# scverse/scanpy

Hardware: AMD Instinct MI355X
Metric: cells/sec through pca+neighbors+leiden, 1M x 2k CSR (higher is better)
Workload: dtype bf16x3

## Files before the change

### include/scanpy_amd.h

```cpp
#ifndef SCANPY_AMD_H
#define SCANPY_AMD_H

#include <stddef.h>
#include <stdint.h>

#ifdef __cplusplus
extern "C" {
#endif

typedef struct ihipStream_t* scamd_stream_t;

#define SCAMD_OK 0
#define SCAMD_EINVAL (-1)
#define SCAMD_EWORKSPACE (-2)
#define SCAMD_EHIP (-3)
#define SCAMD_EUNSUPPORTED (-4)
#define SCAMD_ECAPACITY (-5)
#define SCAMD_EINTERNAL (-6)

#define SCAMD_ABI_VERSION 1

int scamd_abi_version(void);
const char* scamd_last_error(void);
int scamd_device_count(void);
// ... 5 lines not shown
                     double cert_scale, int64_t* n_fallback_host,
                     void* workspace, size_t workspace_bytes, scamd_stream_t stream);
int scamd_knn_l2_ivf_f32(const float* x, int64_t n, int d, int64_t ld_x,
                         int64_t q_begin, int64_t n_query, int k, int nprobe,
                         int32_t* out_idx, double* out_dist, int64_t* n_fallback_host,
                         void* workspace, size_t workspace_bytes, scamd_stream_t stream);
float scamd_knn_last_select_ms(void);
double scamd_knn_last_select_pairs(void);
double scamd_knn_last_select_prepass_pairs(void);
int scamd_knn_last_select_engine(void);
int scamd_knn_last_second_tier_queries(void);
int scamd_knn_last_nprobe(void);
int scamd_knn_last_coarse(void);
void scamd_knn_cert_factors(int engine, double* cert_k, double* cert_k2, double* key_slack);
size_t scamd_knn_debug_b3_scores_workspace_bytes(int64_t n);
int scamd_knn_debug_b3_scores_f32(const float* x, int64_t n, int d, int64_t ld_x, int64_t q0, int nq, int64_t c0, int nc,
                                  float* out_scores, float* out_mu, float* out_cmax, void* workspace,
                                  size_t workspace_bytes, scamd_stream_t stream);
int scamd_knn_debug_cell_tables_sizes(int64_t n, int d, int64_t n_query, int k, int nprobe, int* n_cells, int64_t* n_img_max);
int scamd_knn_debug_cell_tables(int64_t n, int d, int64_t n_query, int k, int nprobe, const void* workspace,
                                size_t workspace_bytes, int32_t* out_labels, int32_t* out_row_cell, int32_t* out_cell_map,
                                float* out_cent, float* out_radius, int32_t* out_tile0, int32_t* out_ntiles, int32_t* out_order,
                                float* out_lb2, int32_t* out_perm, int64_t* n_img_rows_host, scamd_stream_t stream);

size_t scamd_fuzzy_workspace_bytes(int64_t n, int k);
int scamd_fuzzy_simplicial_set_f32(const int32_t* knn_idx, const float* knn_dist, int64_t n, int k,
                                   int64_t* out_indptr, int32_t* out_indices, float* out_data,
                                   int64_t cap, float* out_sigma, float* out_rho, int64_t* nnz_host,
                                   void* workspace, size_t workspace_bytes, scamd_stream_t stream);
int scamd_fuzzy_weights_f32(const int32_t* knn_idx, const float* knn_dist, int64_t n_local, int k, int64_t row_begin,
                            int64_t n_total, const double* sum_all_dev, float* w, float* out_sigma, float* out_rho,
                            int32_t* out_count, scamd_stream_t stream);
size_t scamd_fuzzy_merge_workspace_bytes(int64_t n_local, int64_t cap);
int scamd_fuzzy_merge_rows_f32(const int32_t* knn_idx, const float* w, int64_t n_local, int k, const int64_t* in_indptr,
                               const int32_t* in_src, const float* in_w, int64_t* out_indptr, int32_t* out_indices,
                               float* out_data, int64_t cap, int64_t* nnz_host, void* workspace, size_t workspace_bytes,
                               scamd_stream_t stream);
int scamd_gauss_connectivities_f32(const int32_t* knn_idx, const float* knn_dist, int64_t n, int k, int64_t* out_indptr,
                                   int32_t* out_indices, float* out_data, int64_t cap, int64_t* nnz_host,
                                   void* workspace, size_t workspace_bytes, scamd_stream_t stream);
int scamd_jaccard_connectivities_f32(const int32_t* knn_idx, int64_t n, int k, int64_t* out_indptr,
                                     int32_t* out_indices, float* out_data, int64_t cap, int64_t* nnz_host,
                                     void* workspace, size_t workspace_bytes, scamd_stream_t stream);


int scamd_csr_row_stats_f32(const int64_t* indptr, const float* data, int64_t n_rows,
// ... 236 lines not shown
```

### scanpy_amd/_lib.py

```python
from __future__ import annotations

import ctypes as C
from functools import lru_cache
from pathlib import Path

LIB_PATH = Path(__file__).resolve().parent / "_lib" / "libscanpy_amd.so"

_i64, _i32, _f64, _sz, _vp, _u64 = C.c_int64, C.c_int, C.c_double, C.c_size_t, C.c_void_p, C.c_uint64

SIGNATURES = {
    "scamd_abi_version": (_i32, []),
    "scamd_last_error": (C.c_char_p, []),
    "scamd_device_count": (_i32, []),
    "scamd_knn_workspace_bytes": (_sz, [_i64, _i32, _i64, _i32]),
    "scamd_knn_l2_f32": (_i32, [_vp, _i64, _i32, _i64, _i64, _i64, _i32, _vp, _vp, _f64, C.POINTER(_i64), _vp, _sz, _vp]),
    "scamd_knn_l2_ivf_f32": (_i32, [_vp, _i64, _i32, _i64, _i64, _i64, _i32, _i32, _vp, _vp, C.POINTER(_i64), _vp, _sz, _vp]),
    "scamd_knn_last_select_ms": (C.c_float, []),
    "scamd_knn_last_select_pairs": (_f64, []),
    "scamd_knn_last_select_prepass_pairs": (_f64, []),
    "scamd_knn_last_select_engine": (_i32, []),
    "scamd_knn_last_second_tier_queries": (_i32, []),
    "scamd_knn_last_nprobe": (_i32, []),
    "scamd_knn_last_coarse": (_i32, []),
    "scamd_knn_cert_factors": (None, [_i32, C.POINTER(_f64), C.POINTER(_f64), C.POINTER(_f64)]),
    "scamd_knn_debug_b3_scores_workspace_bytes": (_sz, [_i64]),
    "scamd_knn_debug_b3_scores_f32": (_i32, [_vp, _i64, _i32, _i64, _i64, _i32, _i64, _i32, _vp, _vp, _vp, _vp, _sz, _vp]),
    "scamd_knn_debug_cell_tables_sizes": (_i32, [_i64, _i32, _i64, _i32, _i32, C.POINTER(_i32), C.POINTER(_i64)]),
    "scamd_knn_debug_cell_tables": (_i32, [_i64, _i32, _i64, _i32, _i32, _vp, _sz, _vp, _vp, _vp, _vp, _vp, _vp, _vp, _vp, _vp, _vp,
                                           C.POINTER(_i64), _vp]),
    "scamd_fuzzy_workspace_bytes": (_sz, [_i64, _i32]),
    "scamd_fuzzy_simplicial_set_f32": (_i32, [_vp, _vp, _i64, _i32, _vp, _vp, _vp, _i64, _vp, _vp, C.POINTER(_i64), _vp, _sz, _vp]),
    "scamd_fuzzy_weights_f32": (_i32, [_vp, _vp, _i64, _i32, _i64, _i64, _vp, _vp, _vp, _vp, _vp, _vp]),
    "scamd_fuzzy_merge_workspace_bytes": (_sz, [_i64, _i64]),
    "scamd_fuzzy_merge_rows_f32": (_i32, [_vp, _vp, _i64, _i32, _vp, _vp, _vp, _vp, _vp, _vp, _i64, C.POINTER(_i64), _vp, _sz, _vp]),
    "scamd_gauss_connectivities_f32": (_i32, [_vp, _vp, _i64, _i32, _vp, _vp, _vp, _i64, C.POINTER(_i64), _vp, _sz, _vp]),
    "scamd_jaccard_connectivities_f32": (_i32, [_vp, _i64, _i32, _vp, _vp, _vp, _i64, C.POINTER(_i64), _vp, _sz, _vp]),
    "scamd_csr_row_stats_f32": (_i32, [_vp, _vp, _i64, _vp, _vp, _vp]),
    "scamd_csr_transpose_workspace_bytes": (_sz, [_i64, _i64, _i64]),
    "scamd_csr_transpose_f32": (_i32, [_vp, _vp, _vp, _i64, _i64, _i64, _vp, _vp, _vp, _vp, _sz, _vp]),
    "scamd_spmm_csr_f32": (_i32, [_vp, _vp, _vp, _i64, _i64, _vp, _i32, _vp, _vp, _vp]),
    "scamd_spmm_f64acc_workspace_bytes": (_sz, [_i64, _i64, _i32]),
    "scamd_spmm_csr_f32_f64acc": (_i32, [_vp, _vp, _vp, _i64, _i64, _vp, _i32, _vp, _vp, _vp, _vp, _sz, _vp]),
    "scamd_csr_gram_workspace_bytes": (_sz, [_i64, _i64]),
    "scamd_csr_gram_f32": (_i32, [_vp, _vp, _vp, _i64, _i64, _i64, _i32, _vp, _i64, _vp, C.POINTER(C.c_float), _vp, _sz, _vp]),
    "scamd_eigh_topk_workspace_bytes": (_sz, [_i64, _i32]),
    "scamd_eigh_topk_f64": (_i32, [_vp, _i64, _i64, _i32, _u64, _f64, _vp, _vp, _vp, _vp, _sz, _vp]),
    "scamd_dense_debug_f64": (_i32, [_i32, _vp, _vp, _i32, _i32, _i32, _vp, _vp, C.POINTER(_i32), _vp]),
    "scamd_pca_csr_workspace_bytes": (_sz, [_i64, _i64, _i32]),
    "scamd_pca_csr_f32": (_i32, [_vp, _vp, _vp, _i64, _i64, _i64, _i32, _i32, _u64, _f64, _vp, _vp, _vp, _vp, _vp, _vp, _vp, _sz, _vp]),
    "scamd_pca_solve_gram_workspace_bytes": (_sz, [_i64, _i32]),
    "scamd_pca_solve_gram_f64": (_i32, [_vp, _i64, _vp, _i64, _i64, _i32, _i32, _i32, _u64, _f64, _vp, _vp, _vp, _vp, _vp, _vp, _vp, _vp, _vp, _sz, _vp]),
    "scamd_spectral_embedding_workspace_bytes": (_sz, [_i64, _i64, _i32]),
# ... 131 lines not shown
```

### scanpy_amd/csrc/knn.hip

```cpp
#include "common.h"

#include <algorithm>
#include <cmath>
#include <cstdlib>
#include <memory>
#include <type_traits>
#include <vector>

struct KnnLast {
  float select_ms = -1.f;
  double select_pairs = -1.0, select_prepass_pairs = -1.0;
  int select_engine = -1, second_tier = 0;
  int coarse = 0;
  int nprobe = 0;
};
static thread_local KnnLast g_last;

namespace scamd {

using f32x16 = __attribute__((ext_vector_type(16))) float;
using f32x4 = __attribute__((ext_vector_type(4))) float;
using i32x4 = __attribute__((ext_vector_type(4))) int;
typedef __attribute__((__vector_size__(8 * sizeof(__bf16)))) __bf16 bf16x8;

// ... 989 lines not shown
      } else {
        __syncthreads();
        if (threadIdx.x == 0) {
          int got = -1;
          const int x0 = (int)(blockIdx.x & 7);
          for (int t = 0; t < 8 && got < 0; ++t) {
            const int x = (x0 + t) & 7;
            const int64_t peek = 8 * (int64_t)__hip_atomic_load(&iv.queue_ctr[x], __ATOMIC_RELAXED, __HIP_MEMORY_SCOPE_AGENT) + x;
            if (peek >= iv.n_slots || iv.block_perm[peek] < 0) continue;
            const int64_t slot = 8 * (int64_t)atomicAdd(&iv.queue_ctr[x], 1) + x;
            if (slot < iv.n_slots) got = iv.block_perm[slot];
          }
          *s_next = got;
        }
        __syncthreads();
        blk = *s_next;
      }
      if (blk < 0) return;
      knn_select_reg_block<H, TC_, WPS, IVF, B3, COARSE>(blk, xp, n_tiles_all, n_pad, q_begin, thr_rank, cand_idx, cand_tau, iv);
    }
  }
}

__global__ __launch_bounds__(256) void ivf_cell_order_kernel(const float* __restrict__ centers, int d,
                                                             const float* __restrict__ radius,
                                                             const int* __restrict__ cell_ntiles, int n_cells,
                                                             int* __restrict__ order_out, float* __restrict__ lb2_out,
                                                             int* __restrict__ work_out, int nprobe) {
  extern __shared__ __attribute__((aligned(16))) float co_smem[];
  int npow = 1;
  while (npow < n_cells) npow <<= 1;
  float* lb2 = co_smem;
  int* order = reinterpret_cast<int*>(co_smem + npow);
  const int a = blockIdx.x, tid = threadIdx.x;
  const float ra = radius[a];
  for (int b = tid; b < npow; b += 256) {
    float v = INFINITY;
    if (b < n_cells && cell_ntiles[b] > 0) {
      float d2 = 0.f;
      for (int c = 0; c < d; ++c) {
        const float df = centers[a * d + c] - centers[b * d + c];
        d2 += df * df;
      }
      const float lb = fmaxf(0.f, sqrtf(d2) * (1.0f - 1e-4f) - ra - radius[b]);
      v = (b == a) ? -1.0f : (nprobe > 0 ? d2 : lb * lb);
    }
    lb2[b] = v;
    order[b] = b;
  }
  __syncthreads();
  for (int kk = 2; kk <= npow; kk <<= 1) {
    for (int j = kk >> 1; j > 0; j >>= 1) {
      for (int i = tid; i < npow; i += 256) {
        const int p = i ^ j;
        if (p > i) {
          const bool up = (i & kk) == 0;
          const float vi = lb2[i], vp = lb2[p];
          const int oi = order[i], op = order[p];
          const bool gt = vi > vp || (vi == vp && oi > op);
          if (gt == up) {
            lb2[i] = vp;
            lb2[p] = vi;
            order[i] = op;
            order[p] = oi;
          }
        }
      }
      __syncthreads();
    }
  }
  if (nprobe > 0) {
    for (int i = tid; i < npow; i += 256)
      if (i > 0) lb2[i] = (i < nprobe && lb2[i] < INFINITY) ? 0.f : INFINITY;
    __syncthreads();
  }
  for (int i = tid; i < n_cells; i += 256) {
    order_out[(int64_t)a * n_cells + i] = order[i];
    lb2_out[(int64_t)a * n_cells + i] = lb2[i];
  }
  __shared__ int s_work;
  if (tid == 0) s_work = 0;
  __syncthreads();
  int wsum = 0;
  for (int i = tid; i < n_cells; i += 256)
    if (lb2[i] <= ra * ra) wsum += cell_ntiles[order[i]];
  atomicAdd(&s_work, wsum);
  __syncthreads();
  if (tid == 0) work_out[a] = cell_ntiles[a] > 0 ? s_work : 0;
}

__global__ __launch_bounds__(1024) void ivf_block_order_kernel(const int* __restrict__ work, const int* __restrict__ blk_off,
                                                               const int* __restrict__ blk_cnt, int n_cells,
                                                               int* __restrict__ block_perm, int n_slots, int xcd_mode,
                                                               int* __restrict__ err) {
  __shared__ long long key[IVF_MAX_CELLS];
  __shared__ int start[IVF_MAX_CELLS];
  const int tid = threadIdx.x;
  start[tid] = -1;
  key[tid] = tid < n_cells ? (((long long)(0x7fffffff - work[tid])) << 32) | (unsigned int)tid : 0x7fffffffffffffffll;
  for (int t = tid; t < n_slots; t += 1024) block_perm[t] = -1;
  __syncthreads();
  for (int kk = 2; kk <= IVF_MAX_CELLS; kk <<= 1) {
    for (int j = kk >> 1; j > 0; j >>= 1) {
      const int p = tid ^ j;
      if (p > tid) {
        const bool up = (tid & kk) == 0;
        const long long a = key[tid], b = key[p];
        if ((a > b) == up) {
          key[tid] = b;
          key[p] = a;
        }
// ... 789 lines not shown
  p->n_cells = 0;
  p->n_img_max = p->n_slot_max = 0;
  if (p->ivf) {
    const int cell_rows = std::max(256, env_int("SCAMD_KNN_CELL_ROWS", 2048));
    int c = 16;
    while (c < IVF_MAX_CELLS && (int64_t)c * cell_rows < n) c <<= 1;
    while (c > 1 && (int64_t)c * 256 > n) c >>= 1;
    p->n_cells = c;
    p->n_img_max = (n + (int64_t)64 * c + 255) / 256 * 256;
    p->n_slot_max = n_query + (int64_t)128 * c;
    p->n_pad = p->n_img_max;
  }
  return true;
}

struct KnnBuffers {
  float* xp; float* cn; float* mu; double* mean_partial; unsigned int* cmax; int* cand_idx; float* cand_tau; double* kth_d2;
  int* flag_list; int* counters; double* scratch_d; int* scratch_i; int* fb_counts;
  int* fb_retry[2];
  int* kth_idx;
  int* labels; int* perm; int* qpos; int* block_cell; float* cent; float* centp; long long* sums; int* cell_ints;
  unsigned int* radius_bits; int* cell_order; float* cell_lb2; int* cell_aux; int* block_perm;
  int* qorder;
  int* qrow; float* xp2; int* flag_list2; int* t2_cell; int* t2_pos; int* t2_ints;
};

static size_t block_perm_capacity(const KnnPlan& p) { return (size_t)(p.n_slot_max / 128 + 1) * 2 + 64; }
static void knn_carve(Workspace& ws, const KnnPlan& p, int64_t n_query, KnnBuffers* b) {
  *b = KnnBuffers{};
  b->xp = ws.take<float>((size_t)p.n_pad * p.row_dwords);
  b->cn = ws.take<float>((size_t)p.n_pad);
  b->mu = ws.take<float>(KNN_MAX_D);
  b->mean_partial = ws.take<double>((size_t)MEAN_BLOCKS * KNN_MAX_D);
  b->cmax = ws.take<unsigned int>(4);
  b->cand_idx = ws.take<int>((size_t)p.nq_pad * p.KP);
  b->cand_tau = ws.take<float>((size_t)p.nq_pad);
  b->kth_d2 = ws.take<double>((size_t)n_query);
  b->flag_list = ws.take<int>((size_t)n_query);
  b->counters = ws.take<int>(16);
  b->scratch_d = ws.take<double>((size_t)FALLBACK_CHUNK * FALLBACK_CAP);
  b->scratch_i = ws.take<int>((size_t)FALLBACK_CHUNK * FALLBACK_CAP);
  b->fb_counts = ws.take<int>((size_t)FALLBACK_CHUNK);
  b->fb_retry[0] = ws.take<int>((size_t)n_query);
  b->fb_retry[1] = ws.take<int>((size_t)n_query);
  b->kth_idx = ws.take<int>((size_t)n_query);
  if (p.ivf) {
    b->labels = ws.take<int>((size_t)p.n_pad);
    b->perm = ws.take<int>((size_t)p.n_img_max);
    b->qpos = ws.take<int>((size_t)p.n_slot_max);
    b->block_cell = ws.take<int>((size_t)(p.n_slot_max / 128 + 1));
    b->cent = ws.take<float>((size_t)p.n_cells * 128);
    b->centp = ws.take<float>((size_t)p.n_cells * 136);
    b->sums = ws.take<long long>((size_t)p.n_cells * 128);
    b->cell_ints = ws.take<int>((size_t)p.n_cells * 8);
    b->radius_bits = ws.take<unsigned int>((size_t)p.n_cells);
    b->cell_order = ws.take<int>((size_t)p.n_cells * p.n_cells);
    b->cell_lb2 = ws.take<float>((size_t)p.n_cells * p.n_cells);
    b->cell_aux = ws.take<int>((size_t)p.n_cells * 3);
    b->block_perm = ws.take<int>(block_perm_capacity(p));
    b->qorder = ws.take<int>((size_t)p.n_slot_max);
  }
  if (p.ivf && p.b3) {
    b->qrow = ws.take<int>((size_t)n_query);
    b->xp2 = ws.take<float>((size_t)p.n_img_max * RegCfg<25>::DPL);
    b->flag_list2 = ws.take<int>((size_t)n_query);
    b->t2_cell = ws.take<int>((size_t)n_query);
    b->t2_pos = ws.take<int>((size_t)n_query);
    b->t2_ints = ws.take<int>((size_t)p.n_cells * 2 + 8);
  }
}

struct CellTables {
  int *counts, *qcounts;
  int* cell_map;
  int *row_off, *row_cur;
  int *slot_off, *slot_cur;
  int *tile0, *ntiles;
  const float* radius;
  int *work, *first_block, *n_blocks;
};
static CellTables cell_tables(const KnnBuffers& b, size_t nc) {
  int* const ci = b.cell_ints;
  int* const ca = b.cell_aux;
// ... 60 lines not shown
      case 16: return launch_select_reg<16>(p, b, q_begin, s);
      case 25: return launch_select_reg<25>(p, b, q_begin, s);
      default: return launch_select_reg<32>(p, b, q_begin, s);
    }
  }
  switch (p.H) {
    case 8: return dispatch_kp<8, 128>(p, b, q_begin, s);
    case 16: return dispatch_kp<16, 128>(p, b, q_begin, s);
    case 25: return dispatch_kp<25, 128>(p, b, q_begin, s);
    case 32: return dispatch_kp<32, 128>(p, b, q_begin, s);
    case 64: return dispatch_kp<64, 64>(p, b, q_begin, s);
    default: return dispatch_kp<128, 32>(p, b, q_begin, s);
  }
}

struct KnnCall { const float* x; int64_t n; int d; int64_t ld, q_begin, n_query; hipStream_t s;
                 int k; double cert_scale; int32_t* out_idx; double* out_dist; };
struct HipRelease {
  void operator()(hipEvent_t e) const { (void)hipEventDestroy(e); }
  void operator()(void* p) const { (void)hipFree(p); }
};
using EventOwner = std::unique_ptr<std::remove_pointer_t<hipEvent_t>, HipRelease>;

static IvfArgs ivf_args(const KnnBuffers& b, const CellTables& t, int n_cells, int d) {
  IvfArgs iv{};
  iv.qpos = b.qpos;
  iv.block_cell = b.block_cell;
  iv.cell_tile0 = t.tile0;
  iv.cell_ntiles = t.ntiles;
  iv.centers = b.cent;
  iv.radius = t.radius;
  iv.order = b.cell_order;
  iv.order_lb2 = b.cell_lb2;
  iv.perm = b.perm;
  iv.cmax_bits = b.cmax;
  iv.n_cells = n_cells;
  iv.dc = d;
  iv.d = d;
  iv.block_perm = b.block_perm;
  return iv;
}

static int64_t layout_query_blocks(const std::vector<int>& n_queries, std::vector<int>* slot_off, std::vector<int>* block_cell) {
  int64_t slots = 0;
  for (size_t c = 0; c < n_queries.size(); ++c) {
    slot_off->push_back((int)slots);
    const int nb = (n_queries[c] + 127) / 128;
    block_cell->insert(block_cell->end(), nb, (int)c);
    slots += (int64_t)nb * 128;
  }
  return slots;
}

struct CellLayout {
  std::vector<int> cell_map, row_off, slot_off, tile0, ntiles, block_cell;
  std::vector<int> blocks;
  int64_t rows = 0, slots = 0;
  int n_launch = 0, xcd_mode = 0;
};

static CellLayout ivf_cell_layout(const std::vector<int>& h_cnt, const std::vector<float>& h_cent, int nc, int d, size_t launch_cap) {
  constexpr int MIN_CELL = 128;
  CellLayout L;
  L.cell_map.resize(nc);
  std::vector<int> mc(nc, 0), mq(nc, 0);
  int biggest = 0;
  for (int c = 1; c < nc; ++c)
    if (h_cnt[c] > h_cnt[biggest]) biggest = c;
  for (int c = 0; c < nc; ++c) {
    int tgt = c;
    if (h_cnt[c] < MIN_CELL) {
      tgt = biggest;
      double bestd = INFINITY;
      for (int e = 0; e < nc; ++e) {
        if (h_cnt[e] < MIN_CELL) continue;
        double dd = 0.0;
        for (int t = 0; t < d; ++t) {
          const double df = (double)h_cent[(size_t)c * d + t] - (double)h_cent[(size_t)e * d + t];
          dd += df * df;
        }
        if (dd < bestd) {
          bestd = dd;
          tgt = e;
        }
      }
    }
    L.cell_map[c] = tgt;
    mc[tgt] += h_cnt[c];
    mq[tgt] += h_cnt[nc + c];
  }
  for (int c = 0; c < nc; ++c) {
    L.row_off.push_back((int)L.rows);
    L.tile0.push_back((int)(L.rows / 64));
    L.ntiles.push_back((mc[c] + 63) / 64);
    L.rows += (int64_t)L.ntiles[c] * 64;
  }
  L.slots = layout_query_blocks(mq, &L.slot_off, &L.block_cell);
  L.blocks.resize(2 * nc);
  int maxb = 0;
  for (int c = 0; c < nc; ++c) {
    L.blocks[c] = L.slot_off[c] / 128;
    L.blocks[nc + c] = (mq[c] + 127) / 128;
    maxb = std::max(maxb, L.blocks[nc + c]);
  }
  const int n_blocks = (int)L.block_cell.size();
  const int64_t want = (int64_t)8 * (2 * ((n_blocks + 7) / 8) + maxb);
  L.n_launch = n_blocks;
  if (n_blocks >= 64 && want <= (int64_t)launch_cap) {
    L.xcd_mode = 1;
    L.n_launch = (int)want;
  }
  return L;
}

struct IvfSelect {
  const KnnPlan& p;
  const KnnBuffers& b;
  const KnnCall& c;
  decltype(&ivf_assign_kernel<8>) assign_f32;
  decltype(&knn_select_reg_kernel<8, 64, 3, true, false>) sweep[2];
  size_t sweep_lds;
  const CellTables t = cell_tables(b, p.n_cells);
  const int nc = p.n_cells;
  bool mfma_assign = false;
  int ncp = 0;
  size_t lds_a = 0;
  int assign(int64_t a_start, int64_t a_step, int64_t a_count, int accumulate, int64_t aq0, int64_t aq1, int* a_qcounts,
             bool count_in_kernel = true) const {
    hipStream_t s = c.s;
    if (mfma_assign) {
      unsigned int* centb = reinterpret_cast<unsigned int*>(b.centp);
      hipLaunchKernelGGL(ivf_centpad_bf16_kernel, dim3((unsigned)ceil_div((int64_t)ncp * 32, 256)), dim3(256), 0, s, b.cent, nc, ncp, c.d,
                         centb);
      SCAMD_LAUNCH_CHECK();
      hipLaunchKernelGGL(ivf_assign_mfma_kernel, dim3((unsigned)ceil_div(a_count, ASSIGN_ROWS)), dim3(256), lds_a, s, c.x, c.d, c.ld, a_start,
                         a_step, a_count, centb, ncp, nc, b.labels, count_in_kernel ? t.counts : (int*)nullptr, aq0, aq1, a_qcounts);
      SCAMD_LAUNCH_CHECK();
      if (accumulate) {
        hipLaunchKernelGGL(ivf_sums_kernel, dim3((unsigned)ceil_div(a_count * c.d, 256)), dim3(256), 0, s, c.x, c.d, c.ld, a_start, a_step,
                           a_count, b.labels, b.sums);
        SCAMD_LAUNCH_CHECK();
      }
// ... 26 lines not shown
      hipLaunchKernelGGL(ivf_update_kernel, dim3((unsigned)ceil_div((int64_t)nc * c.d, 256)), dim3(256), 0, c.s, b.sums, t.counts, nc,
                         c.d, b.cent);
      SCAMD_LAUNCH_CHECK();
    }
    return SCAMD_OK;
  }
  int assign_rows(std::vector<int>* h_cnt, std::vector<float>* h_cent) const {
    SCAMD_HIP_CHECK(hipMemsetAsync(t.counts, 0, sizeof(int) * 2 * nc, c.s));
    if (int rc = assign(0, 1, c.n, 0, c.q_begin, c.q_begin + c.n_query, t.qcounts, !mfma_assign)) return rc;
    if (mfma_assign) {
      hipLaunchKernelGGL(ivf_count_kernel, dim3((unsigned)ceil_div(c.n, 4096)), dim3(1024), 0, c.s, b.labels, c.n, nc, c.q_begin,
                         c.q_begin + c.n_query, t.counts, t.qcounts);
      SCAMD_LAUNCH_CHECK();
    }
    SCAMD_HIP_CHECK(hipMemcpyAsync(h_cnt->data(), t.counts, sizeof(int) * 2 * nc, hipMemcpyDeviceToHost, c.s));
    SCAMD_HIP_CHECK(hipMemcpyAsync(h_cent->data(), b.cent, sizeof(float) * nc * c.d, hipMemcpyDeviceToHost, c.s));
    SCAMD_HIP_CHECK(hipStreamSynchronize(c.s));
    return SCAMD_OK;
  }
  int upload_tables(const CellLayout& L) const {
    hipStream_t s = c.s;
    const size_t cell_bytes = sizeof(int) * nc;
    const std::pair<int*, const std::vector<int>*> per_cell[] = {
        {t.cell_map, &L.cell_map}, {t.row_off, &L.row_off}, {t.slot_off, &L.slot_off}, {t.tile0, &L.tile0}, {t.ntiles, &L.ntiles}};
    for (const auto& [dst, src] : per_cell) SCAMD_HIP_CHECK(hipMemcpyAsync(dst, src->data(), cell_bytes, hipMemcpyHostToDevice, s));
    SCAMD_HIP_CHECK(hipMemcpyAsync(b.block_cell, L.block_cell.data(), sizeof(int) * L.block_cell.size(), hipMemcpyHostToDevice, s));
    SCAMD_HIP_CHECK(hipMemcpyAsync(t.first_block, L.blocks.data(), 2 * cell_bytes, hipMemcpyHostToDevice, s));
    SCAMD_HIP_CHECK(hipMemsetAsync(t.row_cur, 0, cell_bytes, s));
    SCAMD_HIP_CHECK(hipMemsetAsync(t.slot_cur, 0, cell_bytes, s));
    SCAMD_HIP_CHECK(hipMemsetAsync(b.perm, 0xff, sizeof(int) * L.rows, s));
    SCAMD_HIP_CHECK(hipMemsetAsync(b.qpos, 0xff, sizeof(int) * L.slots, s));
    SCAMD_HIP_CHECK(hipMemsetAsync(b.radius_bits, 0, sizeof(unsigned int) * nc, s));
    SCAMD_HIP_CHECK(hipMemsetAsync(b.counters + KC_PAIRS, 0, sizeof(int) * (KC_LAUNCH_ORDER_ERR - KC_PAIRS), s));
    SCAMD_HIP_CHECK(hipStreamSynchronize(s));
    return SCAMD_OK;
  }
  int build_image_and_orders(const CellLayout& L) const {
    hipStream_t s = c.s;
    hipLaunchKernelGGL(ivf_scatter_kernel, dim3((unsigned)ceil_div(c.n, 1024 * SCATTER_ROWS)), dim3(1024), 0, s, b.labels, c.n, t.cell_map,
                       t.row_off, t.row_cur, c.q_begin, c.q_begin + c.n_query, t.slot_off, t.slot_cur, b.perm, b.qpos, b.qrow, nc);
    SCAMD_LAUNCH_CHECK();
    const int blocks = (int)std::min<int64_t>((L.rows + 15) / 16, 256 * 16);
    hipLaunchKernelGGL(ivf_pack_image_kernel, dim3(blocks), dim3(256), 0, s, c.x, b.mu, c.d, c.ld, p.H, (p.H + 1 + 3) / 4 * 4, p.row_dwords, L.rows, b.perm, b.labels,
                       t.cell_map, b.cent, b.xp, b.cmax, b.radius_bits, p.b3 ? 1 : 0);
    SCAMD_LAUNCH_CHECK();
    int npow = 1;
    while (npow < nc) npow <<= 1;
    const size_t olds = (size_t)npow * 8;
    SCAMD_HIP_CHECK(hipFuncSetAttribute(reinterpret_cast<const void*>(ivf_cell_order_kernel),
                                        hipFuncAttributeMaxDynamicSharedMemorySize, (int)olds));
    hipLaunchKernelGGL(ivf_cell_order_kernel, dim3(nc), dim3(256), olds, s, b.cent, c.d, t.radius, t.ntiles, nc, b.cell_order, b.cell_lb2,
                       t.work, p.nprobe);
    SCAMD_LAUNCH_CHECK();
    hipLaunchKernelGGL(ivf_block_order_kernel, dim3(1), dim3(1024), 0, s, t.work, t.first_block, t.n_blocks, nc, b.block_perm, L.n_launch,
                       L.xcd_mode, b.counters + KC_LAUNCH_ORDER_ERR);
    SCAMD_LAUNCH_CHECK();
    return SCAMD_OK;
  }
  int choose_coarse(const CellLayout& L, bool* coarse) const {
    *coarse = p.b3 && env_is("SCAMD_KNN_COARSE", '1');
    if (!p.b3 || *coarse || env_is("SCAMD_KNN_COARSE", '0')) return SCAMD_OK;
    std::vector<int> h_work(nc);
    SCAMD_HIP_CHECK(hipMemcpyAsync(h_work.data(), t.work, sizeof(int) * nc, hipMemcpyDeviceToHost, c.s));
    SCAMD_HIP_CHECK(hipStreamSynchronize(c.s));
    double num = 0.0, den = 0.0;
    for (int cell = 0; cell < nc; ++cell) {
      num += (double)L.blocks[nc + cell] * (double)h_work[cell] * 64.0;
      den += (double)L.blocks[nc + cell];
    }
    *coarse = den > 0.0 && num / den >= 5.0e5;
    return SCAMD_OK;
  }
  int launch_sweep(const CellLayout& L, bool coarse, hipEvent_t ev0, hipEvent_t ev1) const {
    hipStream_t s = c.s;
    const size_t n_blocks = L.block_cell.size();
    const auto kern = sweep[coarse];
    const size_t lds = sweep_lds + 64 + IVF_META_BYTES;
    SCAMD_HIP_CHECK(hipFuncSetAttribute(reinterpret_cast<const void*>(kern), hipFuncAttributeMaxDynamicSharedMemorySize, (int)lds));
    IvfArgs iv = ivf_args(b, t, nc, c.d);
    iv.pairs = reinterpret_cast<unsigned long long*>(b.counters + KC_PAIRS);
    iv.qorder = b.qorder;
    iv.prepass_tiles = p.b3 ? 32 : 16;
    iv.prepass_min2 = env_is("SCAMD_KNN_PREPASS_MIN2", '0') ? 0 : 1;
    std::unique_ptr<void, HipRelease> trace;
    const char* trace_path = getenv("SCAMD_KNN_TRACE");
    if (trace_path && trace_path[0]) {
      SCAMD_HIP_CHECK(hipMalloc(reinterpret_cast<void**>(&iv.trace), sizeof(unsigned long long) * 8 * n_blocks));
      trace.reset(iv.trace);
      SCAMD_HIP_CHECK(hipMemsetAsync(iv.trace, 0, sizeof(unsigned long long) * 8 * n_blocks, s));
    }
    int n_groups = L.n_launch;
    iv.n_slots = L.n_launch;
    const int want = env_int("SCAMD_KNN_PERSISTENT", 768);
    if (want > 0 && L.n_launch > want) {
      n_groups = (want + 7) / 8 * 8;
      iv.queue_ctr = b.counters + KC_XCD_QUEUE;
      SCAMD_HIP_CHECK(hipMemsetAsync(b.counters + KC_XCD_QUEUE, 0, sizeof(int) * 8, s));
    }
    SCAMD_HIP_CHECK(hipEventRecord(ev0, s));
    hipLaunchKernelGGL(kern, dim3(n_groups), dim3(RegCfg<8>::NT), lds, s, b.xp, (int)(L.rows / 64), L.rows, c.q_begin, p.thr_rank,
                       b.cand_idx, b.cand_tau, iv);
    SCAMD_LAUNCH_CHECK();
// ... 14 lines not shown
  int run(hipEvent_t ev0, hipEvent_t ev1, int64_t* rows_out) {
    std::vector<int> h_cnt(2 * nc);
    std::vector<float> h_cent((size_t)nc * c.d);
    if (int rc = train_quantiser()) return rc;
    if (int rc = assign_rows(&h_cnt, &h_cent)) return rc;
    const CellLayout L = ivf_cell_layout(h_cnt, h_cent, nc, c.d, block_perm_capacity(p));
    SCAMD_REQUIRE(L.rows <= p.n_img_max && L.slots <= p.n_slot_max, SCAMD_EWORKSPACE, "knn: cell layout exceeds its bound");
    rows_out[0] = L.rows;
    rows_out[1] = L.slots;
    if (L.block_cell.empty()) return SCAMD_OK;
    if (int rc = upload_tables(L)) return rc;
    if (int rc = build_image_and_orders(L)) return rc;
    bool coarse = false;
    if (int rc = choose_coarse(L, &coarse)) return rc;
    g_last.coarse = coarse ? 1 : 0;
    return launch_sweep(L, coarse, ev0, ev1);
  }
};

template <int H, bool B3 = false>
static int run_ivf_select(const KnnPlan& p, const KnnBuffers& b, const KnnCall& c, hipEvent_t ev0, hipEvent_t ev1, int64_t* rows_out) {
  using C = RegCfg<H, 64, B3>;
  static_assert(C::NT == RegCfg<8>::NT, "every instantiation is launched with the same block size");
  IvfSelect sel{p, b, c, ivf_assign_kernel<H>,
                {knn_select_reg_kernel<H, 64, 3, true, B3>, knn_select_reg_kernel<H, 64, 3, true, B3, B3>}, C::LDS_BYTES};
  return sel.run(ev0, ev1, rows_out);
}

static int dispatch_ivf(const KnnPlan& p, const KnnBuffers& b, const KnnCall& c, hipEvent_t ev0, hipEvent_t ev1, int64_t* rows_out) {
  switch (p.H) {
    case 8: return run_ivf_select<8>(p, b, c, ev0, ev1, rows_out);
    case 16: return run_ivf_select<16>(p, b, c, ev0, ev1, rows_out);
    case 25: return p.b3 ? run_ivf_select<25, true>(p, b, c, ev0, ev1, rows_out) : run_ivf_select<25>(p, b, c, ev0, ev1, rows_out);
    default: return run_ivf_select<32>(p, b, c, ev0, ev1, rows_out);
  }
}

static int launch_rerank_rows(const KnnBuffers& b, const KnnCall& c, int thr_rank, double cert_k, double cert_k2, int* flag_list,
                              int* n_flag, const int* qlist, int64_t n_list) {
  const int n_rank = std::max(1, thr_rank - 1);
  const size_t lds = rerank_rows_lds_bytes(c.d, n_rank);
  SCAMD_HIP_CHECK(hipFuncSetAttribute(reinterpret_cast<const void*>(knn_rerank_rows_kernel),
                                      hipFuncAttributeMaxDynamicSharedMemorySize, (int)lds));
  hipLaunchKernelGGL(knn_rerank_rows_kernel, dim3((unsigned)ceil_div(n_list, 8)), dim3(256), lds, c.s, c.x, b.mu, c.n, c.d, c.ld,
                     c.q_begin, c.n_query, c.k, n_rank, b.cand_idx, b.cand_tau, b.cmax, c.cert_scale, cert_k, cert_k2, c.out_idx,
                     c.out_dist, b.kth_d2, flag_list, n_flag, qlist, n_list);
  SCAMD_LAUNCH_CHECK();
// ... 37 lines not shown
  const int n_blocks = (int)h_block_cell.size();
  if (n_blocks == 0) return SCAMD_OK;
  SCAMD_REQUIRE(slots <= p.n_slot_max, SCAMD_EWORKSPACE, "knn: second-tier query layout exceeds its bound");
  SCAMD_HIP_CHECK(hipMemcpyAsync(slot_off2, h_slot_off.data(), sizeof(int) * nc, hipMemcpyHostToDevice, s));
  SCAMD_HIP_CHECK(hipMemcpyAsync(b.block_cell, h_block_cell.data(), sizeof(int) * n_blocks, hipMemcpyHostToDevice, s));
  SCAMD_HIP_CHECK(hipMemsetAsync(b.qpos, 0xff, sizeof(int) * slots, s));
  SCAMD_HIP_CHECK(hipStreamSynchronize(s));
  hipLaunchKernelGGL(ivf_t2_fill_kernel, dim3((unsigned)ceil_div(n_flag, 256)), dim3(256), 0, s, b.flag_list, n_flag, b.t2_cell,
                     b.t2_pos, slot_off2, b.qrow, b.qpos);
  SCAMD_LAUNCH_CHECK();
  t2_dbg(s, __LINE__);
  hipLaunchKernelGGL(knn_iota_kernel, dim3((unsigned)ceil_div(n_blocks, 256)), dim3(256), 0, s, b.block_perm, n_blocks);
  SCAMD_LAUNCH_CHECK();
  t2_dbg(s, __LINE__);
  const int blocks = (int)std::min<int64_t>((rows + 3) / 4, 256 * 16);
  hipLaunchKernelGGL(ivf_pack_image_kernel, dim3(blocks), dim3(256), 0, s, c.x, b.mu, c.d, c.ld, 25, C::HP, C::DPL, rows, b.perm,
                     b.labels, t.cell_map, b.cent, b.xp2, b.cmax, b.radius_bits, 0);
  SCAMD_LAUNCH_CHECK();
  t2_dbg(s, __LINE__);
  auto kern = knn_select_reg_kernel<25, 64, 3, true, false>;
  const size_t lds = C::LDS_BYTES + 64 + IVF_META_BYTES;
  SCAMD_HIP_CHECK(hipFuncSetAttribute(reinterpret_cast<const void*>(kern), hipFuncAttributeMaxDynamicSharedMemorySize,
                                      (int)lds));
  IvfArgs iv = ivf_args(b, t, nc, c.d);
  iv.pairs = reinterpret_cast<unsigned long long*>(ctr2 + KC_PAIRS);
  iv.prepass_tiles = 16;
  iv.prepass_min2 = 1;
  iv.n_slots = n_blocks;
  const int thr_rank = std::min(32, std::max(1, c.k + 6));
  hipLaunchKernelGGL(kern, dim3(n_blocks), dim3(C::NT), lds, s, b.xp2, (int)(rows / 64), rows, c.q_begin, thr_rank, b.cand_idx,
                     b.cand_tau, iv);
  SCAMD_LAUNCH_CHECK();
  t2_dbg(s, __LINE__);
  if (int rc = launch_rerank_rows(b, c, thr_rank, CERT_K_F32, 0.0, b.flag_list2, ctr2 + KC_UNCERTIFIED, b.flag_list, n_flag)) return rc;
  t2_dbg(s, __LINE__);
  SCAMD_READBACK_NOW(n_flag2_host, ctr2 + KC_UNCERTIFIED, sizeof(int), s);
  return SCAMD_OK;
}

static int stage_mean_and_image(const KnnPlan& p, const KnnBuffers& b, const KnnCall& c) {
  hipStream_t s = c.s;
  SCAMD_HIP_CHECK(hipMemsetAsync(b.cmax, 0, 16, s));
  SCAMD_HIP_CHECK(hipMemsetAsync(b.counters, 0, sizeof(int) * KC_HOST_SLOTS, s));
  hipLaunchKernelGGL(knn_colsum_kernel, dim3(MEAN_BLOCKS), dim3(1024), 0, s, c.x, c.n, c.d, c.ld, b.mean_partial);
  SCAMD_LAUNCH_CHECK();
  hipLaunchKernelGGL(knn_colmean_kernel, dim3(1), dim3(KNN_MAX_D), 0, s, b.mean_partial, c.n, c.d, b.mu);
  SCAMD_LAUNCH_CHECK();
// ... 289 lines not shown
  }
  const int64_t rows = ((int64_t)last[0] + last[1]) * 64;
  SCAMD_REQUIRE(last[0] >= 0 && last[1] >= 0 && rows <= n_img_max, SCAMD_EINTERNAL,
                "knn debug cell tables: %lld image rows exceed the plan's %lld (is this the workspace of the same call?)", (long long)rows,
                (long long)n_img_max);
  *n_img_rows_host = rows;
  const size_t cell_bytes = sizeof(int) * (size_t)nc;
  const auto d2d = [&](void* dst, const void* src, size_t bytes) { return hipMemcpyAsync(dst, src, bytes, hipMemcpyDeviceToDevice, s); };
  SCAMD_HIP_CHECK(d2d(out_labels, b.labels, sizeof(int) * (size_t)n));
  SCAMD_HIP_CHECK(d2d(out_cell_map, t.cell_map, cell_bytes));
  SCAMD_HIP_CHECK(d2d(out_cent, b.cent, sizeof(float) * (size_t)nc * d));
  SCAMD_HIP_CHECK(d2d(out_radius, t.radius, cell_bytes));
  SCAMD_HIP_CHECK(d2d(out_tile0, t.tile0, cell_bytes));
  SCAMD_HIP_CHECK(d2d(out_ntiles, t.ntiles, cell_bytes));
  SCAMD_HIP_CHECK(d2d(out_order, b.cell_order, cell_bytes * nc));
  SCAMD_HIP_CHECK(d2d(out_lb2, b.cell_lb2, cell_bytes * nc));
  if (rows > 0) SCAMD_HIP_CHECK(d2d(out_perm, b.perm, sizeof(int) * (size_t)rows));
  hipLaunchKernelGGL(scamd::knn_debug_row_cell_kernel, dim3((unsigned)ceil_div(n, 256)), dim3(256), 0, s, b.labels, t.cell_map, n, nc,
                     out_row_cell);
  SCAMD_LAUNCH_CHECK();
  return SCAMD_OK;
}

namespace scamd {
__global__ void mfma_layout_kernel(int* mismatches) {
  const int lane = threadIdx.x & 63;
  const int i = lane & 31, kk = lane >> 5;
  float a = (float)(i + 100 * kk + 1);
  float bval = (float)(3 * i + 7 * kk + 2);
  f32x16 acc;
#pragma unroll
  for (int r = 0; r < 16; ++r) {
    int row = (r & 3) + 8 * (r >> 2) + 4 * kk;
    acc[r] = (float)(1000 * row + i);
  }
  acc = __builtin_amdgcn_mfma_f32_32x32x2f32(a, bval, acc, 0, 0, 0);
  int bad = 0;
#pragma unroll
  for (int r = 0; r < 16; ++r) {
    int row = (r & 3) + 8 * (r >> 2) + 4 * kk;
    int col = i;
    float expect = (float)(1000 * row + col);
    for (int k2 = 0; k2 < 2; ++k2) expect += (float)(row + 100 * k2 + 1) * (float)(3 * col + 7 * k2 + 2);
    if (acc[r] != expect) ++bad;
  }
  if (bad) atomicAdd(mismatches, bad);
// ... 24 lines not shown
```

Baseline: 23.37 million.

## Tighten IVF cell pruning bounds with per-cell directional reach

Result: faster. 23.92 million (median of 6 runs) (+2.3%).

```diff
diff --git a/include/scanpy_amd.h b/include/scanpy_amd.h
--- a/include/scanpy_amd.h
+++ b/include/scanpy_amd.h
@@ -51,6 +51,9 @@
                                 size_t workspace_bytes, int32_t* out_labels, int32_t* out_row_cell, int32_t* out_cell_map,
                                 float* out_cent, float* out_radius, int32_t* out_tile0, int32_t* out_ntiles, int32_t* out_order,
                                 float* out_lb2, int32_t* out_perm, int64_t* n_img_rows_host, scamd_stream_t stream);
+int scamd_knn_debug_sweep_tables(int64_t n, int d, int64_t n_query, int k, int nprobe, const void* workspace,
+                                 size_t workspace_bytes, float* out_reach, int32_t* out_list_len, int32_t* out_sweep_order,
+                                 float* out_sweep_lb2, scamd_stream_t stream);
 
 size_t scamd_fuzzy_workspace_bytes(int64_t n, int k);
 int scamd_fuzzy_simplicial_set_f32(const int32_t* knn_idx, const float* knn_dist, int64_t n, int k,
diff --git a/scanpy_amd/_lib.py b/scanpy_amd/_lib.py
--- a/scanpy_amd/_lib.py
+++ b/scanpy_amd/_lib.py
@@ -28,6 +28,7 @@
     "scamd_knn_debug_cell_tables_sizes": (_i32, [_i64, _i32, _i64, _i32, _i32, C.POINTER(_i32), C.POINTER(_i64)]),
     "scamd_knn_debug_cell_tables": (_i32, [_i64, _i32, _i64, _i32, _i32, _vp, _sz, _vp, _vp, _vp, _vp, _vp, _vp, _vp, _vp, _vp, _vp,
                                            C.POINTER(_i64), _vp]),
+    "scamd_knn_debug_sweep_tables": (_i32, [_i64, _i32, _i64, _i32, _i32, _vp, _sz, _vp, _vp, _vp, _vp, _vp]),
     "scamd_fuzzy_workspace_bytes": (_sz, [_i64, _i32]),
     "scamd_fuzzy_simplicial_set_f32": (_i32, [_vp, _vp, _i64, _i32, _vp, _vp, _vp, _i64, _vp, _vp, C.POINTER(_i64), _vp, _sz, _vp]),
     "scamd_fuzzy_weights_f32": (_i32, [_vp, _vp, _i64, _i32, _i64, _i64, _vp, _vp, _vp, _vp, _vp, _vp]),
diff --git a/scanpy_amd/csrc/knn.hip b/scanpy_amd/csrc/knn.hip
--- a/scanpy_amd/csrc/knn.hip
+++ b/scanpy_amd/csrc/knn.hip
@@ -1035,6 +1035,41 @@
   }
 }
 
+__device__ __forceinline__ void cell_row_sort(float* lb2, int* order, int npow, int tid) {
+  for (int kk = 2; kk <= npow; kk <<= 1) {
+    for (int j = kk >> 1; j > 0; j >>= 1) {
+      for (int i = tid; i < npow; i += 256) {
+        const int p = i ^ j;
+        if (p > i) {
+          const bool up = (i & kk) == 0;
+          const float vi = lb2[i], vp = lb2[p];
+          const int oi = order[i], op = order[p];
+          const bool gt = vi > vp || (vi == vp && oi > op);
+          if (gt == up) {
+            lb2[i] = vp;
+            lb2[p] = vi;
+            order[i] = op;
+            order[p] = oi;
+          }
+        }
+      }
+      __syncthreads();
+    }
+  }
+}
+__device__ __forceinline__ void cell_row_work(const float* lb2, const int* order, const int* __restrict__ cell_ntiles, int n_cells,
+                                              int a, float ra, int tid, int* __restrict__ work_out) {
+  __shared__ int s_work;
+  if (tid == 0) s_work = 0;
+  __syncthreads();
+  int wsum = 0;
+  for (int i = tid; i < n_cells; i += 256)
+    if (lb2[i] <= ra * ra) wsum += cell_ntiles[order[i]];
+  atomicAdd(&s_work, wsum);
+  __syncthreads();
+  if (tid == 0) work_out[a] = cell_ntiles[a] > 0 ? s_work : 0;
+}
+
 __global__ __launch_bounds__(256) void ivf_cell_order_kernel(const float* __restrict__ centers, int d,
                                                              const float* __restrict__ radius,
                                                              const int* __restrict__ cell_ntiles, int n_cells,
@@ -1062,26 +1097,7 @@
     order[b] = b;
   }
   __syncthreads();
-  for (int kk = 2; kk <= npow; kk <<= 1) {
-    for (int j = kk >> 1; j > 0; j >>= 1) {
-      for (int i = tid; i < npow; i += 256) {
-        const int p = i ^ j;
-        if (p > i) {
-          const bool up = (i & kk) == 0;
-          const float vi = lb2[i], vp = lb2[p];
-          const int oi = order[i], op = order[p];
-          const bool gt = vi > vp || (vi == vp && oi > op);
-          if (gt == up) {
-            lb2[i] = vp;
-            lb2[p] = vi;
-            order[i] = op;
-            order[p] = oi;
-          }
-        }
-      }
-      __syncthreads();
-    }
-  }
+  cell_row_sort(lb2, order, npow, tid);
   if (nprobe > 0) {
     for (int i = tid; i < npow; i += 256)
       if (i > 0) lb2[i] = (i < nprobe && lb2[i] < INFINITY) ? 0.f : INFINITY;
@@ -1091,15 +1107,175 @@
     order_out[(int64_t)a * n_cells + i] = order[i];
     lb2_out[(int64_t)a * n_cells + i] = lb2[i];
   }
-  __shared__ int s_work;
-  if (tid == 0) s_work = 0;
+  cell_row_work(lb2, order, cell_ntiles, n_cells, a, ra, tid, work_out);
+}
+
+#ifdef SCAMD_EMU
+constexpr int REACH_DIRS = 4;
+constexpr int REACH_TILES = 2;
+#else
+constexpr int REACH_DIRS = 32;
+constexpr int REACH_TILES = 8;
+#endif
+constexpr int REACH_MIN_LIST = 8, REACH_MAX_LIST = 64;
+constexpr int REACH_ERR_PAD = 4;
+#define REACH_NONE INFINITY
+__global__ __launch_bounds__(256) void ivf_reach_init_kernel(const float* __restrict__ radius, const int* __restrict__ cell_ntiles,
+                                                             int n_cells, const int* __restrict__ order,
+                                                             const float* __restrict__ lb2, float* __restrict__ reach,
+                                                             int* __restrict__ list_len) {
+  __shared__ int s_len[2];
+  const int p = blockIdx.x, tid = threadIdx.x;
+  const int* orow = order + (int64_t)p * n_cells;
+  const float* brow = lb2 + (int64_t)p * n_cells;
+  if (tid < 2) s_len[tid] = 0;
   __syncthreads();
-  int wsum = 0;
-  for (int i = tid; i < n_cells; i += 256)
-    if (lb2[i] <= ra * ra) wsum += cell_ntiles[order[i]];
-  atomicAdd(&s_work, wsum);
+  const float t15 = 1.5f * radius[p];
+  const float t2 = t15 * t15;
+  int near = 0, finite = 0;
+  for (int i = tid; i < n_cells; i += 256) {
+    const float v = brow[i];
+    near += v <= t2 && v < INFINITY;
+    finite += v < INFINITY;
+  }
+  if (near) atomicAdd(&s_len[0], near);
+  if (finite) atomicAdd(&s_len[1], finite);
   __syncthreads();
-  if (tid == 0) work_out[a] = cell_ntiles[a] > 0 ? s_work : 0;
+  const bool no_structure = s_len[0] > REACH_MAX_LIST && 4 * s_len[0] > 3 * s_len[1];
+  const int len = (cell_ntiles[p] > 0 && !no_structure) ? min(max(s_len[0], min(REACH_MIN_LIST, s_len[1])), REACH_MAX_LIST) : 0;
+  if (tid == 0) list_len[p] = len;
+  for (int i = tid; i < n_cells; i += 256) reach[(int64_t)p * n_cells + orow[i]] = i < len ? -INFINITY : REACH_NONE;
+}
+__device__ __forceinline__ void atomic_max_f32(float* addr, float v) {
+  if (v == 0.f) v = 0.f;
+  if (v >= 0.f) atomicMax(reinterpret_cast<int*>(addr), __float_as_int(v));
+  else atomicMin(reinterpret_cast<unsigned int*>(addr), __float_as_uint(v));
+}
+template <int DP>
+__global__ __launch_bounds__(256) void ivf_reach_kernel(const float* __restrict__ x, int d, int64_t ld,
+                                                        const float* __restrict__ centers,
+                                                        const int* __restrict__ cell_tile0,
+                                                        const int* __restrict__ cell_ntiles, int n_cells,
+                                                        const int* __restrict__ perm, const int* __restrict__ order,
+                                                        const int* __restrict__ list_len,
+                                                        const int* __restrict__ reach_chunks, float* __restrict__ reach) {
+  static_assert(DP % 4 == 0 && REACH_DIRS <= 32, "rows are read as float4; a half-wave holds the directions of a pass");
+  __shared__ __attribute__((aligned(16))) float s_x[64][DP];
+  __shared__ int s_src[64];
+  __shared__ float s_max[8][32];
+  const int tid = threadIdx.x, j = tid & 31, slot = tid >> 5;
+  int lo = 0, hi = n_cells - 1;
+  while (lo < hi) {
+    const int mid = (lo + hi + 1) >> 1;
+    if (reach_chunks[mid] <= (int)blockIdx.x) lo = mid;
+    else hi = mid - 1;
+  }
+  const int p = lo;
+  const int t_lo = ((int)blockIdx.x - reach_chunks[p]) * REACH_TILES, t_hi = min(t_lo + REACH_TILES, cell_ntiles[p]);
+  const int len = list_len[p];
+  if (t_lo >= t_hi) return;
+  const int* orow = order + (int64_t)p * n_cells;
+  float* rrow = reach + (int64_t)p * n_cells;
+  const float* cp = centers + p * d;
+  for (int j0 = 0; j0 < len; j0 += REACH_DIRS) {
+    const int nj = min(REACH_DIRS, len - j0);
+    const float* co = centers + (j < nj ? orow[j0 + j] : p) * d;
+    float w[DP];
+#pragma unroll
+    for (int c = 0; c < DP; ++c) w[c] = c < d ? co[c] - cp[c] : 0.f;
+    float m = -INFINITY;
+    const int row4 = tid >> 2;
+    float nx[DP / 4];
+    int nsrc;
+    auto fetch = [&](int t) __attribute__((always_inline)) {
+      nsrc = t < t_hi ? perm[((int64_t)cell_tile0[p] + t) * 64 + row4] : -1;
+#pragma unroll
+      for (int k = 0; k < DP / 4; ++k) {
+        const int c = (tid & 3) + 4 * k;
+        nx[k] = (nsrc >= 0 && c < d) ? x[(int64_t)nsrc * ld + c] - cp[c] : 0.f;
+      }
+    };
+    fetch(t_lo);
+    for (int t = t_lo; t < t_hi; ++t) {
+      __syncthreads();
+      if ((tid & 3) == 0) s_src[row4] = nsrc;
+#pragma unroll
+      for (int k = 0; k < DP / 4; ++k) s_x[row4][(tid & 3) + 4 * k] = nx[k];
+      __syncthreads();
+      fetch(t + 1);
+#pragma unroll 2
+      for (int i = 0; i < 8; ++i) {
+        const int row = i * 8 + slot;
+        float s = 0.f;
+#pragma unroll
+        for (int c = 0; c < DP; c += 4) {
+          const float4 v = *reinterpret_cast<const float4*>(&s_x[row][c]);
+          s = fmaf(v.x, w[c], s);
+          s = fmaf(v.y, w[c + 1], s);
+          s = fmaf(v.z, w[c + 2], s);
+          s = fmaf(v.w, w[c + 3], s);
+        }
+        m = s_src[row] >= 0 ? fmaxf(m, s) : m;
+      }
+    }
+    __syncthreads();
+    s_max[slot][j] = m;
+    __syncthreads();
+    if (tid < nj) {
+      float v = s_max[0][tid];
+      for (int g = 1; g < 8; ++g) v = fmaxf(v, s_max[g][tid]);
+      if (v > -INFINITY) atomic_max_f32(&rrow[orow[j0 + tid]], v);
+    }
+  }
+}
+
+__global__ __launch_bounds__(256) void ivf_sweep_order_kernel(const float* __restrict__ centers, int d,
+                                                              const float* __restrict__ radius,
+                                                              const int* __restrict__ cell_ntiles, int n_cells,
+                                                              const int* __restrict__ order, const float* __restrict__ lb2,
+                                                              const float* __restrict__ reach,
+                                                              int* __restrict__ sweep_order, float* __restrict__ sweep_lb2,
+                                                              int* __restrict__ work_out) {
+  extern __shared__ __attribute__((aligned(16))) float co_smem[];
+  int npow = 1;
+  while (npow < n_cells) npow <<= 1;
+  float* v2 = co_smem;
+  int* ord = reinterpret_cast<int*>(co_smem + npow);
+  const int a = blockIdx.x, tid = threadIdx.x;
+  const float ra = radius[a];
+  for (int i = tid; i < npow; i += 256) {
+    float v = INFINITY;
+    int b = i;
+    if (i < n_cells) {
+      b = order[(int64_t)a * n_cells + i];
+      v = lb2[(int64_t)a * n_cells + i];
+      if (b != a && v < INFINITY) {
+        double w2 = 0.0;
+        for (int c = 0; c < d; ++c) {
+          const double df = (double)centers[b * d + c] - (double)centers[a * d + c];
+          w2 += df * df;
+        }
+        if (w2 > 0.0) {
+          const double w = sqrt(w2), rb = (double)radius[b];
+          const float fab = reach[(int64_t)a * n_cells + b], fba = reach[(int64_t)b * n_cells + a];
+          const double err = (double)(d + REACH_ERR_PAD) * 0x1p-24;
+          const double rab = fab == REACH_NONE ? (double)ra * w : (double)fab + err * (double)ra * w;
+          const double rba = fba == REACH_NONE ? rb * w : (double)fba + err * rb * w;
+          const double gap = (w - (rab + rba) / w) * (1.0 - 1e-6);
+          if (gap > 0.0) v = fmaxf(v, (float)(gap * gap * (1.0 - 1e-6)));
+        }
+      }
+    }
+    v2[i] = v;
+    ord[i] = b;
+  }
+  __syncthreads();
+  cell_row_sort(v2, ord, npow, tid);
+  for (int i = tid; i < n_cells; i += 256) {
+    sweep_order[(int64_t)a * n_cells + i] = ord[i];
+    sweep_lb2[(int64_t)a * n_cells + i] = v2[i];
+  }
+  cell_row_work(v2, ord, cell_ntiles, n_cells, a, ra, tid, work_out);
 }
 
 __global__ __launch_bounds__(1024) void ivf_block_order_kernel(const int* __restrict__ work, const int* __restrict__ blk_off,
@@ -1935,6 +2111,7 @@
   int* labels; int* perm; int* qpos; int* block_cell; float* cent; float* centp; long long* sums; int* cell_ints;
   unsigned int* radius_bits; int* cell_order; float* cell_lb2; int* cell_aux; int* block_perm;
   int* qorder;
+  float* reach; int* list_len; int* reach_chunks; int* sweep_order; float* sweep_lb2;
   int* qrow; float* xp2; int* flag_list2; int* t2_cell; int* t2_pos; int* t2_ints;
 };
 
@@ -1972,6 +2149,11 @@
     b->cell_aux = ws.take<int>((size_t)p.n_cells * 3);
     b->block_perm = ws.take<int>(block_perm_capacity(p));
     b->qorder = ws.take<int>((size_t)p.n_slot_max);
+    b->reach = ws.take<float>((size_t)p.n_cells * p.n_cells);
+    b->list_len = ws.take<int>((size_t)p.n_cells);
+    b->reach_chunks = ws.take<int>((size_t)p.n_cells);
+    b->sweep_order = ws.take<int>((size_t)p.n_cells * p.n_cells);
+    b->sweep_lb2 = ws.take<float>((size_t)p.n_cells * p.n_cells);
   }
   if (p.ivf && p.b3) {
     b->qrow = ws.take<int>((size_t)n_query);
@@ -2078,7 +2260,7 @@
 };
 using EventOwner = std::unique_ptr<std::remove_pointer_t<hipEvent_t>, HipRelease>;
 
-static IvfArgs ivf_args(const KnnBuffers& b, const CellTables& t, int n_cells, int d) {
+static IvfArgs ivf_args(const KnnBuffers& b, const CellTables& t, int n_cells, int d, int nprobe) {
   IvfArgs iv{};
   iv.qpos = b.qpos;
   iv.block_cell = b.block_cell;
@@ -2086,8 +2268,8 @@
   iv.cell_ntiles = t.ntiles;
   iv.centers = b.cent;
   iv.radius = t.radius;
-  iv.order = b.cell_order;
-  iv.order_lb2 = b.cell_lb2;
+  iv.order = nprobe > 0 ? b.cell_order : b.sweep_order;
+  iv.order_lb2 = nprobe > 0 ? b.cell_lb2 : b.sweep_lb2;
   iv.perm = b.perm;
   iv.cmax_bits = b.cmax;
   iv.n_cells = n_cells;
@@ -2111,6 +2293,8 @@
 struct CellLayout {
   std::vector<int> cell_map, row_off, slot_off, tile0, ntiles, block_cell;
   std::vector<int> blocks;
+  std::vector<int> reach_chunks;
+  int n_reach_blocks = 0;
   int64_t rows = 0, slots = 0;
   int n_launch = 0, xcd_mode = 0;
 };
@@ -2150,6 +2334,8 @@
     L.tile0.push_back((int)(L.rows / 64));
     L.ntiles.push_back((mc[c] + 63) / 64);
     L.rows += (int64_t)L.ntiles[c] * 64;
+    L.reach_chunks.push_back(L.n_reach_blocks);
+    L.n_reach_blocks += (L.ntiles[c] + REACH_TILES - 1) / REACH_TILES;
   }
   L.slots = layout_query_blocks(mq, &L.slot_off, &L.block_cell);
   L.blocks.resize(2 * nc);
@@ -2174,6 +2360,7 @@
   const KnnBuffers& b;
   const KnnCall& c;
   decltype(&ivf_assign_kernel<8>) assign_f32;
+  decltype(&ivf_reach_kernel<16>) reach;
   decltype(&knn_select_reg_kernel<8, 64, 3, true, false>) sweep[2];
   size_t sweep_lds;
   const CellTables t = cell_tables(b, p.n_cells);
@@ -2246,7 +2433,8 @@
     hipStream_t s = c.s;
     const size_t cell_bytes = sizeof(int) * nc;
     const std::pair<int*, const std::vector<int>*> per_cell[] = {
-        {t.cell_map, &L.cell_map}, {t.row_off, &L.row_off}, {t.slot_off, &L.slot_off}, {t.tile0, &L.tile0}, {t.ntiles, &L.ntiles}};
+        {t.cell_map, &L.cell_map}, {t.row_off, &L.row_off}, {t.slot_off, &L.slot_off}, {t.tile0, &L.tile0}, {t.ntiles, &L.ntiles},
+        {b.reach_chunks, &L.reach_chunks}};
     for (const auto& [dst, src] : per_cell) SCAMD_HIP_CHECK(hipMemcpyAsync(dst, src->data(), cell_bytes, hipMemcpyHostToDevice, s));
     SCAMD_HIP_CHECK(hipMemcpyAsync(b.block_cell, L.block_cell.data(), sizeof(int) * L.block_cell.size(), hipMemcpyHostToDevice, s));
     SCAMD_HIP_CHECK(hipMemcpyAsync(t.first_block, L.blocks.data(), 2 * cell_bytes, hipMemcpyHostToDevice, s));
@@ -2276,6 +2464,19 @@
     hipLaunchKernelGGL(ivf_cell_order_kernel, dim3(nc), dim3(256), olds, s, b.cent, c.d, t.radius, t.ntiles, nc, b.cell_order, b.cell_lb2,
                        t.work, p.nprobe);
     SCAMD_LAUNCH_CHECK();
+    if (p.nprobe == 0) {
+      hipLaunchKernelGGL(ivf_reach_init_kernel, dim3(nc), dim3(256), 0, s, t.radius, t.ntiles, nc, b.cell_order, b.cell_lb2, b.reach,
+                         b.list_len);
+      SCAMD_LAUNCH_CHECK();
+      hipLaunchKernelGGL(reach, dim3(L.n_reach_blocks), dim3(256), 0, s, c.x, c.d, c.ld, b.cent, t.tile0, t.ntiles, nc, b.perm,
+                         b.cell_order, b.list_len, b.reach_chunks, b.reach);
+      SCAMD_LAUNCH_CHECK();
+      SCAMD_HIP_CHECK(hipFuncSetAttribute(reinterpret_cast<const void*>(ivf_sweep_order_kernel),
+                                          hipFuncAttributeMaxDynamicSharedMemorySize, (int)olds));
+      hipLaunchKernelGGL(ivf_sweep_order_kernel, dim3(nc), dim3(256), olds, s, b.cent, c.d, t.radius, t.ntiles, nc, b.cell_order, b.cell_lb2,
+                         b.reach, b.sweep_order, b.sweep_lb2, t.work);
+      SCAMD_LAUNCH_CHECK();
+    }
     hipLaunchKernelGGL(ivf_block_order_kernel, dim3(1), dim3(1024), 0, s, t.work, t.first_block, t.n_blocks, nc, b.block_perm, L.n_launch,
                        L.xcd_mode, b.counters + KC_LAUNCH_ORDER_ERR);
     SCAMD_LAUNCH_CHECK();
@@ -2301,7 +2502,7 @@
     const auto kern = sweep[coarse];
     const size_t lds = sweep_lds + 64 + IVF_META_BYTES;
     SCAMD_HIP_CHECK(hipFuncSetAttribute(reinterpret_cast<const void*>(kern), hipFuncAttributeMaxDynamicSharedMemorySize, (int)lds));
-    IvfArgs iv = ivf_args(b, t, nc, c.d);
+    IvfArgs iv = ivf_args(b, t, nc, c.d, p.nprobe);
     iv.pairs = reinterpret_cast<unsigned long long*>(b.counters + KC_PAIRS);
     iv.qorder = b.qorder;
     iv.prepass_tiles = p.b3 ? 32 : 16;
@@ -2362,7 +2563,7 @@
 static int run_ivf_select(const KnnPlan& p, const KnnBuffers& b, const KnnCall& c, hipEvent_t ev0, hipEvent_t ev1, int64_t* rows_out) {
   using C = RegCfg<H, 64, B3>;
   static_assert(C::NT == RegCfg<8>::NT, "every instantiation is launched with the same block size");
-  IvfSelect sel{p, b, c, ivf_assign_kernel<H>,
+  IvfSelect sel{p, b, c, ivf_assign_kernel<H>, ivf_reach_kernel<(2 * H + 3) / 4 * 4>,
                 {knn_select_reg_kernel<H, 64, 3, true, B3>, knn_select_reg_kernel<H, 64, 3, true, B3, B3>}, C::LDS_BYTES};
   return sel.run(ev0, ev1, rows_out);
 }
@@ -2446,7 +2647,7 @@
   const size_t lds = C::LDS_BYTES + 64 + IVF_META_BYTES;
   SCAMD_HIP_CHECK(hipFuncSetAttribute(reinterpret_cast<const void*>(kern), hipFuncAttributeMaxDynamicSharedMemorySize,
                                       (int)lds));
-  IvfArgs iv = ivf_args(b, t, nc, c.d);
+  IvfArgs iv = ivf_args(b, t, nc, c.d, p.nprobe);
   iv.pairs = reinterpret_cast<unsigned long long*>(ctr2 + KC_PAIRS);
   iv.prepass_tiles = 16;
   iv.prepass_min2 = 1;
@@ -2782,6 +2983,30 @@
   return SCAMD_OK;
 }
 
+extern "C" int scamd_knn_debug_sweep_tables(int64_t n, int d, int64_t n_query, int k, int nprobe, const void* workspace,
+                                            size_t workspace_bytes, float* out_reach, int32_t* out_list_len, int32_t* out_sweep_order,
+                                            float* out_sweep_lb2, scamd_stream_t stream) {
+  int nc = 0;
+  int64_t n_img_max = 0;
+  if (int rc = scamd_knn_debug_cell_tables_sizes(n, d, n_query, k, nprobe, &nc, &n_img_max)) return rc;
+  SCAMD_REQUIRE(nprobe <= 0, SCAMD_EINVAL, "knn debug sweep tables: the approximate mode (nprobe=%d) builds none", nprobe);
+  SCAMD_REQUIRE(workspace && out_reach && out_list_len && out_sweep_order && out_sweep_lb2, SCAMD_EINVAL,
+                "knn debug sweep tables: null pointer");
+  KnnPlan p;
+  knn_plan(n, d, n_query, k, &p, 0);
+  Workspace ws(const_cast<void*>(workspace), workspace_bytes);
+  KnnBuffers b;
+  knn_carve(ws, p, n_query, &b);
+  SCAMD_REQUIRE(ws.ok, SCAMD_EWORKSPACE, "knn debug sweep tables: workspace %zu < required %zu", workspace_bytes, ws.used());
+  hipStream_t s = stream;
+  const size_t cell_bytes = sizeof(int) * (size_t)nc;
+  SCAMD_HIP_CHECK(hipMemcpyAsync(out_reach, b.reach, cell_bytes * nc, hipMemcpyDeviceToDevice, s));
+  SCAMD_HIP_CHECK(hipMemcpyAsync(out_list_len, b.list_len, cell_bytes, hipMemcpyDeviceToDevice, s));
+  SCAMD_HIP_CHECK(hipMemcpyAsync(out_sweep_order, b.sweep_order, cell_bytes * nc, hipMemcpyDeviceToDevice, s));
+  SCAMD_HIP_CHECK(hipMemcpyAsync(out_sweep_lb2, b.sweep_lb2, cell_bytes * nc, hipMemcpyDeviceToDevice, s));
+  return SCAMD_OK;
+}
+
 namespace scamd {
 __global__ void mfma_layout_kernel(int* mismatches) {
   const int lane = threadIdx.x & 63;
```
